# opendilab/DI-engine

Measured on NVIDIA H100. Metric: learner transitions/sec (GAE+ppo_error fwd+bwd, T=128 x B=4096 per GPU), higher is better.
Workload: dtype f32

## Files before the change

di-engine_b200/_lib.py:

```python
import ctypes
import os
from ctypes import c_double, c_int, c_longlong, c_size_t, c_void_p

_HERE = os.path.dirname(os.path.abspath(__file__))
LIB_PATH = os.environ.get("B200RL_LIB") or os.path.join(_HERE, "lib", "libb200rl.so")

P = c_void_p
LL = c_longlong
D = c_double
I = c_int

PROTOTYPES = {
    "b200rl_version": [],
    "b200rl_built_for_sm": [],
    "b200rl_workspace_bytes": [],
    "b200rl_gae": [P, P, P, P, P, P, LL, LL, LL, D, D, I, P],
    "b200rl_gae_returns": [P, P, P, P, P, LL, LL, LL, D, D, I, D, P, P, P, P, P, P, P, c_size_t, P],
    "b200rl_adv_stats": [P, LL, P, P, c_size_t, P],
    "b200rl_normalize": [P, P, LL, P, P],
    "b200rl_gae_returns_norm": [P, P, P, P, P, LL, LL, D, D, I, D, P, P, P, P, P, P, P, P, P, c_size_t, P],
    "b200rl_value_map_fwd": [I, P, LL, P, P],
    "b200rl_value_map_bwd": [I, P, P, LL, P, P],
    "b200rl_impala_mask": [P, P, P, LL, LL, P, P, P, P],
    "b200rl_ppo_fwd": [P, P, P, P, P, P, P, P, P, LL, LL, LL, D, I, D, I, P, P, P, P, c_size_t, P],
    "b200rl_ppo_bwd": [P, P, P, P, P, P, P, P, P, LL, LL, LL, D, I, D, I, P, P, P, P, P, P, P, P, P, P, P],
    "b200rl_ppo_fwd_grad": [P, P, P, P, P, P, P, P, P, LL, LL, LL, D, I, D, I, P, P, P, P, P, P, P, P, c_size_t, P],
    "b200rl_ppo_value_fwd": [P, P, P, P, LL, D, I, P, P, P, c_size_t, P],
    "b200rl_ppo_fused_supported": [P, P, P, P, P, P, P, P, P, P, LL, LL],
    "b200rl_qntd_fwd": [P, P, P, P, P, P, P, P, LL, P, LL, LL, LL, I, D, I, I, D, I, D, I, LL, D, P, P, P, P, P, P, P,
                        c_size_t, P],
    "b200rl_qntd_bwd": [P, P, P, P, P, LL, LL, LL, I, LL, I, P, P],
    "b200rl_dqfd_fwd": [P, P, P, P, P, P, P, P, P, P, P, LL, P, LL, LL, I, D, I, I, D, I, D, D, D, D, D, LL, D, P, P, P,
                        P, P, P, P, P, P, c_size_t, P],
    "b200rl_dqfd_bwd": [P, P, P, P, P, P, P, P, LL, LL, D, D, D, LL, I, P, P],
    "b200rl_soft_td_fwd": [I, P, P, P, P, P, P, P, P, LL, LL, LL, LL, I, D, D, D, I, I, D, P, P, P, P, P, P, P, P, P,
                           c_size_t, P],
    "b200rl_dntd_fwd":[P, P, P, P, P, P, P, LL, P, LL, P, LL, LL, LL, I, I, D, D, D, P, P, P, P, P, P, c_size_t, P],
    "b200rl_dntd_bwd": [P, P, P, P, LL, P, P, LL, LL, I, I, P, P],
    "b200rl_lambda_returns": [P, P, P, D, P, D, P, I, LL, LL, P, P],
    "b200rl_lambda_returns_bwd": [P, P, P, P, P, D, P, D, P, I, LL, LL, P, P, P, P, P],
    "b200rl_tb_cross_entropy_fwd": [P, P, P, LL, LL, LL, P, P],
    "b200rl_tb_cross_entropy_bwd": [P, P, P, P, LL, LL, LL, P, P],
    "b200rl_td_lambda_fwd": [P, P, P, D, D, LL, LL, P, P, P, c_size_t, P],
    "b200rl_scale": [P, P, P, LL, P],
    "b200rl_upgo_head_fwd": [P, P, P, P, P, P, LL, LL, LL, P, P, P, P, c_size_t, P],
    "b200rl_upgo_head_bwd": [P, P, P, P, P, LL, LL, LL, I, P, P],
    "b200rl_vtrace_fwd": [P, P, P, P, P, P, LL, LL, LL, D, D, D, D, D, P, P, P, P, P, c_size_t, P],
    "b200rl_vtrace_continuous_fwd": [P, P, P, P, P, P, P, P, LL, LL, LL, D, D, D, D, D, P, P, P, P, P, c_size_t, P],
    "b200rl_vtrace_continuous_bwd": [P, P, P, P, P, P, P, P, P, LL, LL, LL, P, P, P, P],
    "b200rl_vtrace_fused_supported": [P, P, P, P, P, P, LL, LL, LL, P, P],
    "b200rl_vtrace_fwd_grad": [P, P, P, P, P, P, LL, LL, LL, D, D, D, D, D, P, I, P, P, P, P, P, P, P, P, P, c_size_t, P],
    "b200rl_gae_ppo_supported": [P, P, P, P, P, LL, LL, P, P, P, P, P, P, P, P, LL, P, P],
    "b200rl_gae_ppo_fwd_grad": [P, P, P, P, P, LL, LL, D, D, I, P, P, P, P, P, P, P, P, LL, D, I, D, I, P, P, P, P, P, P,
                                P, c_size_t, P],
    "b200rl_gae_ppo_fwd_grad_dp": [P, P, P, P, P, LL, LL, D, D, I, P, P, P, P, P, P, P, P, LL, D, I, D, I, P, P, P, P, P,
                                   P, P, I, I, P, P, P, c_size_t, P],
    "b200rl_p2p_drain_mean": [P, I, I, I, P, P, P],
    "b200rl_a2c_fwd_grad": [P, P, P, P, P, P, LL, LL, P, I, P, P, P, P, P, P, P, P, P, c_size_t, P],
    "b200rl_ppo_continuous_fwd_grad": [P, P, P, P, P, P, P, P, P, P, P, P, P, LL, LL, D, I, D, I, P, I, P, P, P, P, P, P, P, P, P,
                                       P, P, c_size_t, P],
    "b200rl_a2c_continuous_fwd_grad": [P, P, P, P, P, P, P, LL, LL, P, I, P, P, P, P, P, P, P, P, P, P, c_size_t, P],
    "b200rl_grpo_fwd_grad": [I, P, P, P, P, P, P, LL, LL, LL, D, D, P, P, P, P, P, c_size_t, P],
    "b200rl_rloo_fwd_grad": [I, P, P, P, P, LL, P, LL, LL, LL, D, P, P, P, P, P, c_size_t, P],
    "b200rl_token_logp_fwd": [I, P, P, LL, LL, P, P, P],
    "b200rl_token_logp_bwd": [I, P, P, P, P, P, I, LL, LL, P, P],
    "b200rl_token_head_fwd": [P, P, P, P, P, LL, P, LL, LL, D, D, P, P, P, c_size_t, P],
    "b200rl_ppo_lm_fwd_grad": [I, P, P, P, P, P, P, LL, LL, D, D, I, I, P, P, P, P, P, P, P, P, P, c_size_t, P],
    "b200rl_ppo_lm_bwd": [I, P, P, P, LL, LL, P, P, P, P, P, P, P, P, P, P, P],
    "b200rl_a2c_lm_fwd_grad": [I, P, P, P, P, P, P, LL, LL, P, P, P, P, P, P, P, P, P, P, c_size_t, P],
    "b200rl_a2c_lm_bwd": [I, P, P, P, LL, LL, P, P, P, P, P, P, P, P, P, P, P, P],
    "b200rl_gae_ppo_set_impl": [I],
    "b200rl_vtrace_set_impl": [I],
    "b200rl_acer_policy_fwd": [P, P, P, P, P, P, LL, LL, D, P, P, P],
    "b200rl_acer_policy_bwd": [P, P, P, P, P, P, P, P, LL, LL, D, P, P],
    "b200rl_acer_value_fwd": [P, P, P, LL, LL, P, P],
    "b200rl_acer_value_bwd": [P, P, P, P, LL, LL, P, P],
    "b200rl_acer_trust_region": [P, P, LL, LL, D, P, P],
    "b200rl_ppg_bc_fwd": [P, P, P, LL, LL, P, P, P, c_size_t, P],
    "b200rl_q_retraces": [P, P, P, P, P, P, LL, LL, LL, D, P, P],
    "b200rl_quantile_td_fwd": [P, P, P, P, P, P, P, P, P, LL, LL, LL, LL, LL, LL, D, LL, LL, LL, LL, LL, LL, LL, LL, I, D, P, P,
                               P, P, P, c_size_t, P],
# ... 44 lines not shown
```

di-engine_b200/csrc/colws.cu:

```cuda
#include "../../include/b200rl.h"
#include "fused_args.cuh"

namespace b200rl {

constexpr int CW_CW = 8;
constexpr int CW_CT = CW_CW * 32;
constexpr int CW_THREADS = CW_CT + 64;
template <int TC> struct CwGeo {
    static constexpr int R = CW_CT / TC;
    static constexpr int MAX_STAGES = TC == 32 ? 8 : 4;
    static constexpr int CTAS_PER_SM = TC == 32 ? 1 : 2;
    static constexpr int PR = TC / 4;
    static constexpr int RAW_SLOTS = TC == 32 ? 4 : 2;
};
constexpr int CW_AHEAD = 2;
constexpr int CW_RAW_ARR = CW_CT * 4;
constexpr int CW_RAW_BYTES = 5 * CW_RAW_ARR;

constexpr int CW_TRACE_CHUNKS = 13;
#define CW_TRACE(slot)                                                                                   \
    do {                                                                                                 \
        if (f.trace) reinterpret_cast<unsigned long long*>(ws + 65536)[blockIdx.x * 64 + (slot)] = gtimer(); \
    } while (0)

// ... 356 lines not shown
    const long long S = a.S, L = S * a.N * 4, F = S * 4;
    const ByteSpan s[] = {byte_span(a.logit_new, L), byte_span(a.logit_old, L), byte_span(a.logit_pre, L),
                          byte_span(a.action, S * 8),   byte_span(a.value_new, F), byte_span(a.value_old, F),
                          byte_span(a.ret, F),          byte_span(a.weight, F),    byte_span(f.value, F),
                          byte_span(f.next_value, F),   byte_span(f.reward, F),    byte_span(f.done, F),
                          byte_span(f.traj, F)};
    for (const ByteSpan& x : s) *r++ = x;
    return (int)(sizeof(s) / sizeof(s[0]));
}

static int cw_writes(const FusedArgs& f, float* out, float* ws, size_t ws_bytes, ByteSpan* w) {
    const PpoArgs& a = f.p;
    const long long S = a.S, F = S * 4;
    const ByteSpan s[] = {byte_span(a.adv_out, F),
                          byte_span(a.grad_logit, S * a.N * 4),
                          byte_span(a.grad_value, F),
                          byte_span(f.mask_inplace ? f.next_value : nullptr, F),
                          byte_span(a.rec.used, 4 * sizeof(float)),
                          byte_span(ws, (long long)ws_bytes),
                          byte_span(out, 8 * sizeof(float)),
                          byte_span(f.x_seq, 24 * sizeof(unsigned int)),
                          byte_span(f.x_out_mean, 16 * sizeof(float))};
    for (const ByteSpan& x : s) *w++ = x;
    return (int)(sizeof(s) / sizeof(s[0]));
}

template <int NC, bool GRADS, int TC>
static int launch_ws(const FusedArgs& f_in, float* out, float* ws, size_t ws_bytes, cudaStream_t st) {
    FusedArgs f = f_in;
    const PpoArgs& a = f.p;
    const ChainPoint at = capture_now(st);
    ByteSpan span[16];
    f.defer_wait = !f.x_mailboxes && chain_may_defer(st, at, span, cw_early_reads(f, span));
    const int stages = cw_stages<TC>(f);
    const size_t smem = cw_smem<TC>(a.N, a.logit_pre != nullptr, a.weight != nullptr, stages);
    constexpr auto kern = gae_ppo_ws_kernel<NC, GRADS, TC>;
    int sm_count, per_sm;
    if (int rc = resident_ctas<kern>(CW_THREADS, smem, sm_count, per_sm)) return rc;
    if (per_sm > CwGeo<TC>::CTAS_PER_SM) per_sm = CwGeo<TC>::CTAS_PER_SM;
    const long long n_tiles = (f.B + TC - 1) / TC;
    long long grid = (long long)sm_count * per_sm;
    if (grid > n_tiles) grid = n_tiles;
    if (ws_bytes < WS_MIN_BYTES || !ws_partials_fit((long long)(grid * 6), ws_bytes))
        return B200RL_ERR_WORKSPACE;
    if (int rc = launch_k(kern, (int)grid, CW_THREADS, smem, st, f, ws, stages)) return rc;
    FinalizeArgs fa = ppo_finalize_args(a.S, a.logit_pre != nullptr, (int)grid);
    fa.x.mailboxes = f.x_mailboxes; fa.x.state = f.x_seq; fa.x.out_mean = f.x_out_mean; fa.x.rank = f.x_rank;
    fa.x.world = f.x_world;
    if (int rc = launch_finalize(ws, out, fa, st)) return rc;
    chain_report(st, at, true, span, cw_writes(f, out, ws, ws_bytes, span));
    return B200RL_OK;
}

static int cw_sm_count(int& n) {
    static int sms[MAX_DEVICES];
    int dev = 0;
    if (int rc = current_device(dev)) return rc;
    if (sms[dev] == 0)
        if (int rc = cuda_rc(cudaDeviceGetAttribute(&sms[dev], cudaDevAttrMultiProcessorCount, dev))) return rc;
    n = sms[dev];
    return B200RL_OK;
}

template <bool GRADS>
static int dispatch_ws(const FusedArgs& f, float* out, float* ws, size_t ws_bytes, cudaStream_t st) {
    int sm_count = 0;
    if (int rc = cw_sm_count(sm_count)) return rc;
    const int tc = cw_pick_tc(f, sm_count);
    return with_nc(f.p.N, [&](auto nc) {
        return tc == 32 ? launch_ws<nc, GRADS, 32>(f, out, ws, ws_bytes, st) : launch_ws<nc, GRADS, 16>(f, out, ws, ws_bytes, st);
    });
}

int launch_colws(const FusedArgs& f, bool grads, float* out, float* ws, size_t ws_bytes, cudaStream_t st) {
    return grads ? dispatch_ws<true>(f, out, ws, ws_bytes, st) : dispatch_ws<false>(f, out, ws, ws_bytes, st);
}

}
```

di-engine_b200/csrc/common.cuh:

```cuda
#pragma once
#include <cuda_runtime.h>
#include <stdint.h>
#include <stdlib.h>

#include <type_traits>

#define B200RL_OK 0
#ifndef B200RL_ERR_ARG
#define B200RL_ERR_ARG (-1)
#define B200RL_ERR_WORKSPACE (-2)
#endif

#define WS_CTRL_WORDS 16
#define WS_MIN_BYTES (1u << 20)

namespace b200rl {

constexpr int NUM_SMS = 132;

__device__ __forceinline__ float fmul(float a, float b) { return __fmul_rn(a, b); }
__device__ __forceinline__ float fadd(float a, float b) { return __fadd_rn(a, b); }
__device__ __forceinline__ float fsub(float a, float b) { return __fsub_rn(a, b); }

__device__ __forceinline__ float ldg_stream(const float* p) { return __ldcs(p); }
// ... 499 lines not shown
    UpstreamRecord r{};
    for (int k = 0; k < 4; ++k) r.g[k] = expected ? expected + k : nullptr;
    r.used = used;
    return r;
}

static inline UpstreamRecord verify_record(const float* g0, const float* g1, const float* g2, const float* g3,
                                           const float* used, float* hint) {
    return UpstreamRecord{{g0, g1, g2, g3}, const_cast<float*>(used), hint, 1};
}

__device__ __forceinline__ float upstream_value(const UpstreamRecord& r, unsigned owned, int k) {
    return ((owned >> k) & 1u) && r.g[k] ? *r.g[k] : 0.f;
}

template <int K>
__device__ __forceinline__ bool upstream(const UpstreamRecord& r, bool verify, unsigned owned, float (&g)[K]) {
    const bool cmp = verify && r.used != nullptr;
    bool same = cmp;
#pragma unroll
    for (int k = 0; k < K; ++k) g[k] = upstream_value(r, owned, k);
#pragma unroll
    for (int k = 0; k < K; ++k)
        if (cmp && ((owned >> k) & 1u)) same &= __float_as_uint(g[k]) == __float_as_uint(r.used[k]);
    float* rec = verify ? r.hint : r.used;
    if (rec && blockIdx.x == 0 && threadIdx.x == 0)
#pragma unroll
        for (int k = 0; k < K; ++k)
            if (!verify || ((owned >> k) & 1u)) rec[k] = g[k];
    return same;
}

static inline bool upstream_args_ok(int verify, const float* out, bool grads, bool bufs, const float* expected,
                                    const float* used) {
    return verify ? bufs : (out && (!grads || (bufs && expected && used)));
}

constexpr int MAX_DEVICES = 64;

static inline int current_device(int& dev) {
    if (int rc = cuda_rc(cudaGetDevice(&dev))) return rc;
    return (dev >= 0 && dev < MAX_DEVICES) ? B200RL_OK : B200RL_ERR_ARG;
}

template <auto K>
static inline int smem_opt_in(size_t smem) {
    static size_t opted[MAX_DEVICES];
    if (smem <= 48 * 1024) return B200RL_OK;
    int dev = 0;
    if (int rc = current_device(dev)) return rc;
    if (smem <= opted[dev]) return B200RL_OK;
    if (int rc = cuda_rc(cudaFuncSetAttribute(K, cudaFuncAttributeMaxDynamicSharedMemorySize, (int)smem))) return rc;
    opted[dev] = smem;
    return B200RL_OK;
}

template <auto K>
static inline int resident_ctas(int threads, size_t smem, int& sm_count, int& per_sm) {
    static int sms[MAX_DEVICES];
    static size_t occ_smem[MAX_DEVICES];
    static int occ[MAX_DEVICES];
    if (int rc = smem_opt_in<K>(smem)) return rc;
    int dev = 0;
    if (int rc = current_device(dev)) return rc;
    if (sms[dev] == 0)
        if (int rc = cuda_rc(cudaDeviceGetAttribute(&sms[dev], cudaDevAttrMultiProcessorCount, dev))) return rc;
    if (occ[dev] == 0 || occ_smem[dev] != smem) {
        if (int rc = cuda_rc(cudaOccupancyMaxActiveBlocksPerMultiprocessor(&occ[dev], K, threads, smem))) return rc;
        occ_smem[dev] = smem;
    }
    sm_count = sms[dev];
    per_sm = occ[dev];
    return per_sm < 1 ? B200RL_ERR_ARG : B200RL_OK;
}

template <class F>
static inline int with_nc(int n, F&& f) {
    switch (n) {
        case 2: return f(std::integral_constant<int, 2>{});
        case 3: return f(std::integral_constant<int, 3>{});
        case 4: return f(std::integral_constant<int, 4>{});
        case 5: return f(std::integral_constant<int, 5>{});
        case 6: return f(std::integral_constant<int, 6>{});
        case 7: return f(std::integral_constant<int, 7>{});
        case 8: return f(std::integral_constant<int, 8>{});
        case 9: return f(std::integral_constant<int, 9>{});
        case 10: return f(std::integral_constant<int, 10>{});
        case 12: return f(std::integral_constant<int, 12>{});
        case 14: return f(std::integral_constant<int, 14>{});
        case 16: return f(std::integral_constant<int, 16>{});
        case 18: return f(std::integral_constant<int, 18>{});
        default: return f(std::integral_constant<int, 0>{});
    }
}

struct ByteSpan {
    uintptr_t lo, hi;
};
static inline ByteSpan byte_span(const void* p, long long bytes) {
    const uintptr_t lo = reinterpret_cast<uintptr_t>(p);
    return (p && bytes > 0) ? ByteSpan{lo, lo + (uintptr_t)bytes} : ByteSpan{0, 0};
}

struct ChainPoint {
    int dev;
    bool capturing;
// ... 43 lines not shown
```

di-engine_b200/csrc/ppo.cu:

```cuda
#include "../../include/b200rl.h"
#include "ppo_math.cuh"

namespace b200rl {

template <int NC, int WHAT>
__global__ void __launch_bounds__(PPO_THREADS) ppo_tile_kernel(PpoArgs a, float* out, float* ws) {
    constexpr int PPO_R = PPO_CT;
    pdl_prologue();
    extern __shared__ __align__(128) unsigned char smem[];
    constexpr bool GRADS = (WHAT != PPO_FWD);
    constexpr bool LOSSES = (WHAT != PPO_BWD);
    const int N = NC ? NC : a.N;
    const int tid = threadIdx.x;
    const int wid = tid >> 5, lane = tid & 31;
    const bool is_producer = wid == PPO_CW;
    const bool has_pre = a.logit_pre != nullptr, has_w = a.weight != nullptr;
    const PpoTileLayout L = ppo_layout(N, has_pre, has_w, PPO_R);
    const int warp_out_bytes = 32 * N * 4;
    unsigned char* outbuf = smem + PPO_STAGES * L.stage_bytes;
    uint64_t* full = reinterpret_cast<uint64_t*>(outbuf + (GRADS ? PPO_OUTBUFS * L.logit_bytes : 0));
    uint64_t* empty = full + PPO_STAGES;

    float g[4] = {0.f, 0.f, 0.f, 0.f};
    if (GRADS && upstream<4>(a.rec, WHAT == PPO_BWD, ppo_owned(a), g)) return;
    const PpoUpstream up{g[0], g[1], g[2], g[3], 1.f / (float)a.S};

    const long long n_full = a.S / PPO_R;
    const int tail_rows = (int)(a.S - n_full * PPO_R);
    const long long n_tiles = n_full + (tail_rows ? 1 : 0);
    const int my_n = (n_tiles > blockIdx.x) ? (int)((n_tiles - blockIdx.x + gridDim.x - 1) / gridDim.x) : 0;

    if (tid == 0) {
        for (int s = 0; s < PPO_STAGES; ++s) {
            mbar_init(&full[s], 1);
            mbar_init(&empty[s], PPO_CW);
        }
        mbar_fence_init();
    }
    __syncthreads();

    float acc[6] = {0.f, 0.f, 0.f, 0.f, 0.f, 0.f};
    if (is_producer) {
        if (lane == 0) {
            for (int i = 0; i < my_n; ++i) {
                const long long t = blockIdx.x + (long long)i * gridDim.x;
                if (t >= n_full) break;
                const int sg = i % PPO_STAGES;
                if (i >= PPO_STAGES) mbar_wait(&empty[sg], (uint32_t)(((i / PPO_STAGES) - 1) & 1));
                const long long row0 = t * PPO_R;
                unsigned char* st = smem + sg * L.stage_bytes;
                uint64_t* bar = &full[sg];
                mbar_expect_tx(bar, (uint32_t)L.tx_bytes);
                tma_load_1d(st, a.logit_new + row0 * N, L.logit_bytes, bar);
                tma_load_1d(st + L.off_old, a.logit_old + row0 * N, L.logit_bytes, bar);
                if (has_pre) tma_load_1d(st + L.off_pre, a.logit_pre + row0 * N, L.logit_bytes, bar);
                tma_load_1d(st + L.off_act, a.action + row0, PPO_R * 8, bar);
                tma_load_1d(st + L.off_vn, a.value_new + row0, PPO_R * 4, bar);
                tma_load_1d(st + L.off_vo, a.value_old + row0, PPO_R * 4, bar);
                tma_load_1d(st + L.off_adv, a.adv + row0, PPO_R * 4, bar);
                tma_load_1d(st + L.off_ret, a.ret + row0, PPO_R * 4, bar);
                if (has_w) tma_load_1d(st + L.off_w, a.weight + row0, PPO_R * 4, bar);
            }
        }
    } else {
    const int rit = wid * 32 + lane;
    for (int i = 0; i < my_n; ++i) {
        const long long t = blockIdx.x + (long long)i * gridDim.x;
        const long long row0 = t * PPO_R;
        const int sg = i % PPO_STAGES;
        unsigned char* st = smem + sg * L.stage_bytes;
        const bool full_tile = t < n_full;
        if (full_tile) {
            mbar_wait(&full[sg], (uint32_t)((i / PPO_STAGES) & 1));
        } else {
            if (rit < tail_rows) {
                float* d0 = reinterpret_cast<float*>(st) + rit * N;
                float* d1 = reinterpret_cast<float*>(st + L.off_old) + rit * N;
                float* d2 = reinterpret_cast<float*>(st + L.off_pre) + rit * N;
                for (int k = 0; k < N; ++k) {
                    d0[k] = a.logit_new[(row0 + rit) * N + k];
                    d1[k] = a.logit_old[(row0 + rit) * N + k];
                    if (has_pre) d2[k] = a.logit_pre[(row0 + rit) * N + k];
                }
                reinterpret_cast<long long*>(st + L.off_act)[rit] = a.action[row0 + rit];
                reinterpret_cast<float*>(st + L.off_vn)[rit] = a.value_new[row0 + rit];
                reinterpret_cast<float*>(st + L.off_vo)[rit] = a.value_old[row0 + rit];
                reinterpret_cast<float*>(st + L.off_adv)[rit] = a.adv[row0 + rit];
                reinterpret_cast<float*>(st + L.off_ret)[rit] = a.ret[row0 + rit];
                if (has_w) reinterpret_cast<float*>(st + L.off_w)[rit] = a.weight[row0 + rit];
            }
        }
        float* gtile = reinterpret_cast<float*>(outbuf + (wid * 2 + (i & 1)) * warp_out_bytes) - wid * 32 * N;
        if (full_tile || rit < tail_rows) {
            const float adv = reinterpret_cast<const float*>(st + L.off_adv)[rit];
            ppo_row_compute<NC, LOSSES, GRADS>(a, L, st, rit, N, adv, full_tile, gtile, row0, up, acc);
        }
        if (full_tile) {
            if (GRADS) {
                fence_proxy_async_smem();
                __syncwarp();
                if (lane == 0) {
                    tma_store_1d(a.grad_logit + (row0 + wid * 32) * N, gtile + wid * 32 * N, warp_out_bytes);
                    tma_store_commit();
                    tma_store_wait_read<1>();
                }
            }
            __syncwarp();
            if (lane == 0) mbar_arrive(&empty[sg]);
        }
    }
    if (GRADS && lane == 0) tma_store_wait_read<0>();
    }
    if (LOSSES) grid_store_partials<6, PPO_THREADS>(acc, ws);
}

template <int NT, int MODE>
__global__ void __launch_bounds__(NT) ppo_fwd_kernel(PpoArgs a, float* out, float* ws) {
    pdl_prologue();
    constexpr int L = (MODE == 2) ? 32 : 1;
    const int lane = (MODE == 2) ? (threadIdx.x & 31) : 0;
    const int N = a.N, G = a.G;
    const long long per_cta = (MODE == 1) ? NT : NT / 32;
    long long s = (MODE == 1) ? (long long)blockIdx.x * NT + threadIdx.x
                              : (long long)blockIdx.x * (NT / 32) + (threadIdx.x >> 5);
    float acc[6] = {0.f, 0.f, 0.f, 0.f, 0.f, 0.f};
    for (; s < a.S; s += per_cta * gridDim.x) {
        const float* zn = a.logit_new + s * G * N;
        const float* zo = a.logit_old + s * G * N;
        const float* zp = a.logit_pre ? a.logit_pre + s * G * N : nullptr;
        float ratio_sum = 0.f, ent_sum = 0.f, akl = 0.f, kl = 0.f;
        for (int g = 0; g < G; ++g) {
            const float* rn = zn + (size_t)g * N;
            const float* ro = zo + (size_t)g * N;
            const int act = (int)a.action[s * G + g];
            float lse_n, ent;
            row_lse_entropy<L>([&](int j) { return rn[j]; }, N, lane, lse_n, ent);
            const float lse_o = row_lse<L>([&](int j) { return ro[j]; }, N, lane);
            const float lp_n = rn[act] - lse_n;
            const float lp_o = ro[act] - lse_o;
            ratio_sum += expf(lp_n - lp_o);
            ent_sum += ent;
            akl += lp_o - lp_n;
            if (zp) {
                const float* rp = zp + (size_t)g * N;
                const float lse_p = row_lse<L>([&](int j) { return rp[j]; }, N, lane);
                float dummy;
                kl += kl_term(lp_n - (rp[act] - lse_p), a.kl_type, dummy);
            }
        }
        if (lane == 0) {
            const float w = a.weight ? a.weight[s] : 1.f;
            const float adv = adv_in(a, a.adv[s]);
            const float ratio = (G == 1) ? ratio_sum : ratio_sum / (float)G;
            const float ent = (G == 1) ? ent_sum : ent_sum / (float)G;
            float dsel;
            const float sel = surrogate(ratio, adv, a.clip_lo, a.clip_hi, a.dual_clip, dsel, false, a.factor ? a.factor[s] : 1.f);
            acc[0] -= sel * w;
            float dterm;
            acc[1] += value_term(a.value_new[s], a.value_old[s], a.ret[s], a.clip, a.use_value_clip, dterm) * w;
            acc[2] += ent * w;
            acc[3] += kl;
            acc[4] += akl;
            acc[5] += (ratio > a.clip_hi || ratio < a.clip_lo) ? 1.f : 0.f;
        }
    }
    double tot[6];
// ... 57 lines not shown
        float c_act = g_pol * (-w * inv_s) * dsel * ratio_g / (float)G;
        if (zp) {
            const float* rp = zp + (size_t)g * N;
            const float lse_p = row_lse<L>([&](int j) { return rp[j]; }, N, lane);
            float dk;
            kl_term(lp_n - (rp[act] - lse_p), a.kl_type, dk);
            c_act += g_kl * dk * inv_m;
        }
        const float c_ent = g_ent * w * inv_m;
        for (int j = lane; j < N; j += L) {
            const float lp = fmaxf(rn[j] - lse_n, kF32Min);
            const float p = expf(lp);
            float gj = -c_act * p - c_ent * p * (lp + ent);
            if (j == act) gj += c_act;
            gr[j] = gj;
        }
    }
    if (lane == 0) {
        float dterm;
        value_term(a.value_new[s], a.value_old[s], a.ret[s], a.clip, a.use_value_clip, dterm);
        a.grad_value[s] = g_val * 0.5f * w * inv_s * dterm;
    }
    }
}

static bool tile_path_ok(const PpoArgs& a) {
    const bool al = aligned16(a.logit_new) && aligned16(a.logit_old) && (!a.logit_pre || aligned16(a.logit_pre)) &&
                    aligned16(a.action) && aligned16(a.value_new) && aligned16(a.value_old) && aligned16(a.adv) &&
                    aligned16(a.ret) && (!a.weight || aligned16(a.weight)) &&
                    (!a.grad_logit || aligned16(a.grad_logit));
    return a.G == 1 && a.N <= 32 && al;
}

template <int NT>
__global__ void __launch_bounds__(NT) ppo_value_kernel(const float* __restrict__ value_new,
                                                       const float* __restrict__ value_old,
                                                       const float* __restrict__ ret, const float* __restrict__ weight,
                                                       long long S, float clip, int use_clip, float* __restrict__ out,
                                                       float* __restrict__ dvalue, float* ws) {
    pdl_prologue();
    float acc[1] = {0.f};
    const float inv_s = 1.f / (float)S;
    for (long long i = (long long)blockIdx.x * NT + threadIdx.x; i < S; i += (long long)gridDim.x * NT) {
        const float w = weight ? weight[i] : 1.f;
        float d;
        const float t = value_term(value_new[i], use_clip ? value_old[i] : 0.f, ret[i], clip, use_clip, d);
        acc[0] += t * w;
        if (dvalue) dvalue[i] = 0.5f * w * inv_s * d;
    }
    double tot[1];
    if (grid_sum<1, NT>(acc, tot, ws, 0) && threadIdx.x == 0) out[0] = (float)(0.5 * tot[0] / (double)S);
}

template <int NC, int WHAT>
static int launch_tile(const PpoArgs& a, float* out, float* ws, size_t ws_bytes, cudaStream_t st) {
    constexpr int PPO_R = PPO_CT;
    const PpoTileLayout L = ppo_layout(a.N, a.logit_pre != nullptr, a.weight != nullptr, PPO_R);
    const size_t smem = (size_t)PPO_STAGES * L.stage_bytes + (WHAT != PPO_FWD ? (size_t)PPO_OUTBUFS * L.logit_bytes : 0) +
                        2 * PPO_STAGES * sizeof(uint64_t);
    constexpr auto kern = ppo_tile_kernel<NC, WHAT>;
    if (smem > 227 * 1024) return B200RL_ERR_ARG;
    int sm_count, per_sm;
    if (int rc = resident_ctas<kern>(PPO_THREADS, smem, sm_count, per_sm)) return rc;
    if (per_sm > 6) per_sm = 6;
    const long long n_tiles = (a.S + PPO_R - 1) / PPO_R;
    long long grid = (long long)sm_count * ((WHAT == PPO_BWD && a.rec.used) ? 1 : per_sm);
    if (grid > n_tiles) grid = n_tiles;
    if (WHAT != PPO_BWD && !ws_partials_fit((long long)(grid * 6), ws_bytes)) return B200RL_ERR_WORKSPACE;
    if (int rc = launch_k(kern, (int)grid, PPO_THREADS, smem, st, a, out, ws)) return rc;
    if (WHAT == PPO_BWD) return B200RL_OK;
    return launch_finalize(ws, out, ppo_finalize_args(a.S, a.logit_pre != nullptr, (int)grid), st);
}

template <int WHAT>
static int dispatch_tile(const PpoArgs& a, float* out, float* ws, size_t ws_bytes, cudaStream_t st) {
    return with_nc(a.N, [&](auto nc) { return launch_tile<nc, WHAT>(a, out, ws, ws_bytes, st); });
}

}

using namespace b200rl;

static int fill_args(PpoArgs& a, const float* logit_new, const float* logit_old, const float* logit_pretrained,
                     const long long* action, const float* value_new, const float* value_old, const float* adv,
                     const float* return_, const float* weight, long long S, long long G, long long N,
                     double clip_ratio, int use_value_clip, double dual_clip, int kl_type, const float* adv_stats,
                     const float* factor) {
    a.adv_stats = adv_stats;
    a.factor = factor;
    a.logit_new = logit_new; a.logit_old = logit_old; a.logit_pre = logit_pretrained; a.action = action;
    a.value_new = value_new; a.value_old = value_old; a.adv = adv; a.ret = return_; a.weight = weight;
    a.S = S; a.G = (int)G; a.N = (int)N; a.clip = (float)clip_ratio; a.clip_lo = (float)(1.0 - clip_ratio);
    a.clip_hi = (float)(1.0 + clip_ratio); a.dual_clip = (float)dual_clip;
    a.use_value_clip = use_value_clip; a.kl_type = kl_type;
    if (S < 0 || G < 1 || N < 1) return B200RL_ERR_ARG;
    if (!logit_new || !logit_old || !action || !value_new || !value_old || !adv || !return_) return B200RL_ERR_ARG;
    if (kl_type < 1 || kl_type > 3) return B200RL_ERR_ARG;
    return B200RL_OK;
}

extern "C" int b200rl_ppo_fwd(const float* logit_new, const float* logit_old, const float* logit_pretrained,
                              const long long* action, const float* value_new, const float* value_old,
                              const float* adv, const float* return_, const float* weight, long long S, long long G,
                              long long N, double clip_ratio, int use_value_clip, double dual_clip, int kl_type,
                              const float* adv_stats, const float* factor, float* out, float* workspace,
                              size_t workspace_bytes, void* stream) {
    PpoArgs a{};
    int rc = fill_args(a, logit_new, logit_old, logit_pretrained, action, value_new, value_old, adv, return_, weight,
                       S, G, N, clip_ratio, use_value_clip, dual_clip, kl_type, adv_stats, factor);
    if (rc != B200RL_OK || !out || !workspace) return rc != B200RL_OK ? rc : B200RL_ERR_ARG;
    if (S == 0) return B200RL_ERR_ARG;
    cudaStream_t st = (cudaStream_t)stream;
    if (tile_path_ok(a)) return dispatch_tile<PPO_FWD>(a, out, workspace, workspace_bytes, st);
    constexpr int NT = 128;
    const bool warp = a.N > 64;
    int grid = warp ? div_up(S, NT / 32) : div_up(S, NT);
    if (grid > NUM_SMS * 16) grid = NUM_SMS * 16;
    if (!ws_partials_fit((long long)((size_t)grid * 6), workspace_bytes)) return B200RL_ERR_WORKSPACE;
    if (warp) return launch_k(ppo_fwd_kernel<NT, 2>, grid, NT, 0, st, a, out, workspace);
    return launch_k(ppo_fwd_kernel<NT, 1>, grid, NT, 0, st, a, out, workspace);
}

extern "C" int b200rl_ppo_fwd_grad(const float* logit_new, const float* logit_old, const float* logit_pretrained,
                                   const long long* action, const float* value_new, const float* value_old,
// ... 9 lines not shown
    if (rc != B200RL_OK) return rc;
    if (!workspace || S == 0 || !upstream_args_ok(0, out, true, grad_logit_new && grad_value_new, g_expected, g_used))
        return B200RL_ERR_ARG;
    a.rec = forward_record(g_expected, g_used); a.grad_logit = grad_logit_new; a.grad_value = grad_value_new;
    if (!tile_path_ok(a)) return B200RL_ERR_ARG;
    return dispatch_tile<PPO_FWD_GRAD>(a, out, workspace, workspace_bytes, (cudaStream_t)stream);
}

extern "C" int b200rl_ppo_fused_supported(const float* logit_new, const float* logit_old,
                                          const float* logit_pretrained, const long long* action,
                                          const float* value_new, const float* value_old, const float* adv,
                                          const float* return_, const float* weight, const float* grad_logit_new,
                                          long long G, long long N) {
    PpoArgs a{};
    a.logit_new = logit_new; a.logit_old = logit_old; a.logit_pre = logit_pretrained; a.action = action;
    a.value_new = value_new; a.value_old = value_old; a.adv = adv; a.ret = return_; a.weight = weight;
    a.grad_logit = const_cast<float*>(grad_logit_new); a.G = (int)G; a.N = (int)N;
    return tile_path_ok(a) ? 1 : 0;
}

extern "C" int b200rl_ppo_bwd(const float* logit_new, const float* logit_old, const float* logit_pretrained,
                              const long long* action, const float* value_new, const float* value_old,
                              const float* adv, const float* return_, const float* weight, long long S, long long G,
                              long long N, double clip_ratio, int use_value_clip, double dual_clip, int kl_type,
                              const float* adv_stats, const float* factor, const float* g_policy, const float* g_value,
                              const float* g_entropy, const float* g_kl,
                              const float* g_used, float* g_hint, float* grad_logit_new, float* grad_value_new,
                              void* stream) {
    PpoArgs a{};
    int rc = fill_args(a, logit_new, logit_old, logit_pretrained, action, value_new, value_old, adv, return_, weight,
                       S, G, N, clip_ratio, use_value_clip, dual_clip, kl_type, adv_stats, factor);
    if (rc != B200RL_OK) return rc;
    if (!upstream_args_ok(1, nullptr, true, grad_logit_new && grad_value_new, nullptr, g_used)) return B200RL_ERR_ARG;
    a.rec = verify_record(g_policy, g_value, g_entropy, g_kl, g_used, g_hint);
    a.grad_logit = grad_logit_new; a.grad_value = grad_value_new;
    if (S == 0) return B200RL_OK;
    cudaStream_t st = (cudaStream_t)stream;
    constexpr int NT = 128;
    if (tile_path_ok(a)) {
        const ChainPoint at = capture_now(st);
        if (int rc = dispatch_tile<PPO_BWD>(a, nullptr, nullptr, 0, st)) return rc;
        const ByteSpan w[] = {byte_span(grad_logit_new, S * G * N * 4), byte_span(grad_value_new, S * 4),
                              byte_span(g_hint, 4 * sizeof(float))};
        chain_report(st, at, false, w, 3);
        return B200RL_OK;
    }
    if (g_used) return B200RL_ERR_ARG;
    long long grid = a.N > 64 ? div_up(S, NT / 32) : div_up(S, NT);
    if (grid > NUM_SMS * 32) grid = NUM_SMS * 32;
    if (a.N > 64) return launch_k(ppo_bwd_kernel<NT, 2>, (int)grid, NT, 0, st, a);
    return launch_k(ppo_bwd_kernel<NT, 1>, (int)grid, NT, 0, st, a);
}

extern "C" int b200rl_ppo_value_fwd(const float* value_new, const float* value_old, const float* return_,
                                    const float* weight, long long S, double clip_ratio, int use_value_clip,
                                    float* loss, float* dvalue_unit, float* workspace, size_t workspace_bytes,
                                    void* stream) {
    if (!value_new || !return_ || (use_value_clip && !value_old) || !loss || !workspace || S < 1) return B200RL_ERR_ARG;
    constexpr int NT = 256;
    long long grid = div_up(S, NT);
    if (grid > NUM_SMS * 8) grid = NUM_SMS * 8;
    if (workspace_bytes < WS_MIN_BYTES || !ws_partials_fit((long long)(grid), workspace_bytes))
        return B200RL_ERR_WORKSPACE;
    return launch_k(ppo_value_kernel<NT>, (int)grid, NT, 0, (cudaStream_t)stream, value_new, value_old, return_, weight,
                    S, (float)clip_ratio, use_value_clip, loss, dvalue_unit, workspace);
}
```

include/b200rl.h:

```cpp
#ifndef B200RL_H_
#define B200RL_H_

#include <stddef.h>

#ifdef __cplusplus
extern "C" {
#endif

#if defined(__GNUC__)
#define B200RL_API __attribute__((visibility("default")))
#else
#define B200RL_API
#endif

#define B200RL_ERR_ARG (-1)
#define B200RL_ERR_WORKSPACE (-2)

B200RL_API int b200rl_version(void);
B200RL_API int b200rl_built_for_sm(void);
B200RL_API size_t b200rl_workspace_bytes(void);

B200RL_API int b200rl_gae(const float* value, float* next_value, const float* reward, const float* done, const float* traj_flag,
               float* adv, long long T, long long C, long long A, double gamma, double lambda_,
               int mask_next_value_inplace, void* stream);

B200RL_API int b200rl_gae_returns(const float* value, float* next_value, const float* reward, const float* done,
                       const float* traj_flag, long long T, long long C, long long A, double gamma, double lambda_,
                       int mask_next_value_inplace, double value_scale, float* adv, float* unnormalized_return,
                       float* value_out, float* return_out, float* stats3, float* adv_stats2, float* workspace,
                       size_t workspace_bytes, void* stream);
B200RL_API int b200rl_adv_stats(const float* x, long long n, float* stats2, float* workspace, size_t workspace_bytes,
                     void* stream);
B200RL_API int b200rl_normalize(const float* x, const float* stats2, long long n, float* out, void* stream);

B200RL_API int b200rl_gae_returns_norm(const float* value, const float* next_value, const float* reward, const float* done,
                            const float* traj_flag, long long T, long long C, double gamma, double lambda_,
                            int value_norm, double std, const float* popart_mu, const float* popart_sigma, float* adv,
                            float* value_out, float* return_out, float* stats3, float* adv_stats2, float* scratch,
                            float* workspace, size_t workspace_bytes, void* stream);

B200RL_API int b200rl_value_map_fwd(int mode, const float* x, long long n, float* y, void* stream);
B200RL_API int b200rl_value_map_bwd(int mode, const float* x, const float* g, long long n, float* dx, void* stream);

B200RL_API int b200rl_impala_mask(const float* values, const float* rewards, const float* done, long long T, long long B,
                       float* values_out, float* rewards_out, float* weights_out, void* stream);

B200RL_API int b200rl_ppo_fwd(const float* logit_new, const float* logit_old, const float* logit_pretrained,
                   const long long* action, const float* value_new, const float* value_old, const float* adv,
                   const float* return_, const float* weight, long long S, long long G, long long N,
                   double clip_ratio, int use_value_clip, double dual_clip, int kl_type, const float* adv_stats,
                   const float* factor, float* out, float* workspace, size_t workspace_bytes, void* stream);
B200RL_API int b200rl_ppo_bwd(const float* logit_new, const float* logit_old, const float* logit_pretrained,
                   const long long* action, const float* value_new, const float* value_old, const float* adv,
                   const float* return_, const float* weight, long long S, long long G, long long N,
                   double clip_ratio, int use_value_clip, double dual_clip, int kl_type, const float* adv_stats,
                   const float* factor, const float* g_policy, const float* g_value, const float* g_entropy, const float* g_kl,
                   const float* g_used, float* g_hint, float* grad_logit_new, float* grad_value_new, void* stream);
B200RL_API int b200rl_ppo_fwd_grad(const float* logit_new, const float* logit_old, const float* logit_pretrained,
                        const long long* action, const float* value_new, const float* value_old, const float* adv,
                        const float* return_, const float* weight, long long S, long long G, long long N,
                        double clip_ratio, int use_value_clip, double dual_clip, int kl_type, const float* adv_stats,
                        const float* factor, const float* g_expected, float* g_used, float* out, float* grad_logit_new,
                        float* grad_value_new, float* workspace, size_t workspace_bytes, void* stream);
B200RL_API int b200rl_ppo_fused_supported(const float* logit_new, const float* logit_old, const float* logit_pretrained,
                               const long long* action, const float* value_new, const float* value_old,
                               const float* adv, const float* return_, const float* weight,
                               const float* grad_logit_new, long long G, long long N);

B200RL_API int b200rl_qntd_fwd(const float* q, const float* next_n_q, const long long* action, const long long* next_n_action,
                    const float* reward, const float* done, const float* weight, const float* value_gamma,
                    long long value_gamma_stride, const float* gamma_per_sample, long long S, long long G, long long N,
                    int nstep, double gamma, int cum_reward, int rescale, double rescale_eps, int criterion,
                    double criterion_param, int group_mean, long long seq_len, double priority_mix, float* loss,
                    float* td_error_per_sample, float* dcrit_saved, float* target_out, float* grad_q_unit,
                    float* priority_out, float* workspace, size_t workspace_bytes, void* stream);
B200RL_API int b200rl_qntd_bwd(const float* dcrit_saved, const float* weight, const long long* action, const float* g_loss,
                    const float* g_td, long long S, long long G, long long N, int group_mean, long long seq_len,
                    int skip_if_unit, float* grad_q, void* stream);

B200RL_API int b200rl_dqfd_fwd(const float* q, const float* next_n_q, const float* new_n_q_one_step, const long long* action,
                    const long long* next_n_action, const long long* next_n_action_one_step, const float* reward,
                    const float* done, const float* done_one_step, const float* weight, const float* value_gamma,
                    long long value_gamma_stride, const float* is_expert, long long S, long long N, int nstep,
                    double gamma, int cum_reward, int rescale, double rescale_eps, int criterion, double criterion_param,
                    double lambda_n_step_td, double lambda_one_step_td, double lambda_supervised_loss, double margin,
                    long long seq_len, double priority_mix, float* loss, float* td_error_per_sample,
                    float* loss_statistics, float* saved, float* target_n_out, float* target_1_out, float* grad_q_unit,
                    float* priority_out, float* workspace, size_t workspace_bytes, void* stream);
B200RL_API int b200rl_dqfd_bwd(const float* saved, const float* weight, const long long* action, const float* g_loss,
                    const float* g_td, const float* g_loss_statistics_n, const float* g_loss_statistics_1,
                    const float* g_loss_statistics_je, long long S, long long N, double lambda_n_step_td,
                    double lambda_one_step_td, double lambda_supervised_loss, long long seq_len, int skip_if_unit,
                    float* grad_q, void* stream);

B200RL_API int b200rl_soft_td_fwd(int mode, const float* q, const float* target_q, const float* next_q, const long long* action,
                       const float* reward, const float* done, const float* weight, const float* value_gamma,
                       long long value_gamma_stride, long long S, long long G, long long N, int nstep, double gamma,
                       double tau, double alpha, int cum_reward, int criterion, double criterion_param, float* loss,
                       float* td_error_per_sample, float* dcrit_saved, float* target_out, float* grad_q_unit,
                       float* action_gap, float* clipfrac, float* record_target_v, float* workspace,
                       size_t workspace_bytes, void* stream);

B200RL_API int b200rl_dntd_fwd(const float* dist, const float* next_n_dist, const long long* act, const long long* next_n_act,
                    const float* reward, const float* done, const float* weight, long long weight_stride,
                    const float* value_gamma, long long value_gamma_stride, const float* support, long long B,
                    long long A, long long N, int n_atom, int nstep, double gamma, double v_min, double v_max,
                    float* loss, float* td_error_per_sample, float* proj_saved, int* bad_flag, float* grad_dist_unit,
                    float* workspace, size_t workspace_bytes, void* stream);
B200RL_API int b200rl_dntd_bwd(const float* dist, const long long* act, const float* proj_saved, const float* weight,
                    long long weight_stride, const float* g_loss, const float* g_td, long long R, long long N,
                    int n_atom, int skip_if_unit, float* grad_dist, void* stream);

B200RL_API int b200rl_lambda_returns(const float* value, const float* reward, const float* gammas, double gamma,
                          const float* lambdas, double lambda_, const float* done, int upgo_mode, long long T,
                          long long B, float* ret, void* stream);
B200RL_API int b200rl_lambda_returns_bwd(const float* g_ret, const float* value, const float* reward, const float* ret,
// ... 194 lines not shown
```

Baseline: 21.31 billion.

## Restructure PPO tile kernel into one persistent CTA per SM with deep pipeline

Rewrites the PPO tile kernel so each SM runs a single persistent CTA that takes a contiguous range of tiles. Stage count is sized dynamically to fill shared memory, and the producer limits itself to a fixed prefetch distance. Gradients are written in place into the input stage buffer instead of separate output buffers, and the stage is released only after the TMA store has read it. It also adds optional per-CTA timer tracing and a geometry query API. The goal is deeper load/compute overlap and less smem overhead, but it risks lower occupancy and less latency hiding than several CTAs per SM. It is also unclear whether the workload's fused GAE+PPO path uses this kernel at all.

```diff
diff --git a/di-engine_b200/_lib.py b/di-engine_b200/_lib.py
--- a/di-engine_b200/_lib.py
+++ b/di-engine_b200/_lib.py
@@ -27,6 +27,7 @@
     "b200rl_ppo_fwd_grad": [P, P, P, P, P, P, P, P, P, LL, LL, LL, D, I, D, I, P, P, P, P, P, P, P, P, c_size_t, P],
     "b200rl_ppo_value_fwd": [P, P, P, P, LL, D, I, P, P, P, c_size_t, P],
     "b200rl_ppo_fused_supported": [P, P, P, P, P, P, P, P, P, P, LL, LL],
+    "b200rl_ppo_tile_geometry": [LL, LL, I, I, I, I, P],
     "b200rl_qntd_fwd": [P, P, P, P, P, P, P, P, LL, P, LL, LL, LL, I, D, I, I, D, I, D, I, LL, D, P, P, P, P, P, P, P,
                         c_size_t, P],
     "b200rl_qntd_bwd": [P, P, P, P, P, LL, LL, LL, I, LL, I, P, P],
diff --git a/di-engine_b200/csrc/colws.cu b/di-engine_b200/csrc/colws.cu
--- a/di-engine_b200/csrc/colws.cu
+++ b/di-engine_b200/csrc/colws.cu
@@ -432,20 +432,10 @@
     return B200RL_OK;
 }
 
-static int cw_sm_count(int& n) {
-    static int sms[MAX_DEVICES];
-    int dev = 0;
-    if (int rc = current_device(dev)) return rc;
-    if (sms[dev] == 0)
-        if (int rc = cuda_rc(cudaDeviceGetAttribute(&sms[dev], cudaDevAttrMultiProcessorCount, dev))) return rc;
-    n = sms[dev];
-    return B200RL_OK;
-}
-
 template <bool GRADS>
 static int dispatch_ws(const FusedArgs& f, float* out, float* ws, size_t ws_bytes, cudaStream_t st) {
     int sm_count = 0;
-    if (int rc = cw_sm_count(sm_count)) return rc;
+    if (int rc = sm_count_of(sm_count)) return rc;
     const int tc = cw_pick_tc(f, sm_count);
     return with_nc(f.p.N, [&](auto nc) {
         return tc == 32 ? launch_ws<nc, GRADS, 32>(f, out, ws, ws_bytes, st) : launch_ws<nc, GRADS, 16>(f, out, ws, ws_bytes, st);
diff --git a/di-engine_b200/csrc/common.cuh b/di-engine_b200/csrc/common.cuh
--- a/di-engine_b200/csrc/common.cuh
+++ b/di-engine_b200/csrc/common.cuh
@@ -575,6 +575,16 @@
     if (smem <= opted[dev]) return B200RL_OK;
     if (int rc = cuda_rc(cudaFuncSetAttribute(K, cudaFuncAttributeMaxDynamicSharedMemorySize, (int)smem))) return rc;
     opted[dev] = smem;
+    return B200RL_OK;
+}
+
+static inline int sm_count_of(int& n) {
+    static int sms[MAX_DEVICES];
+    int dev = 0;
+    if (int rc = current_device(dev)) return rc;
+    if (sms[dev] == 0)
+        if (int rc = cuda_rc(cudaDeviceGetAttribute(&sms[dev], cudaDevAttrMultiProcessorCount, dev))) return rc;
+    n = sms[dev];
     return B200RL_OK;
 }
 
diff --git a/di-engine_b200/csrc/ppo.cu b/di-engine_b200/csrc/ppo.cu
--- a/di-engine_b200/csrc/ppo.cu
+++ b/di-engine_b200/csrc/ppo.cu
@@ -3,77 +3,96 @@
 
 namespace b200rl {
 
+constexpr int PS_CW = 8;
+constexpr int PS_R = PS_CW * 32;
+constexpr int PS_THREADS = PS_R + 32;
+constexpr int PS_MAX_STAGES = 8;
+constexpr int PS_AHEAD = 2;
+constexpr size_t PS_SMEM_LIMIT = 227 * 1024 - 1024;
+constexpr int PS_TRACE_STAGES = 56;
+
 template <int NC, int WHAT>
-__global__ void __launch_bounds__(PPO_THREADS) ppo_tile_kernel(PpoArgs a, float* out, float* ws) {
-    constexpr int PPO_R = PPO_CT;
+__global__ void __launch_bounds__(PS_THREADS, 1) ppo_tile_kernel(PpoArgs a, float* ws, int n_stages, int trace) {
+    extern __shared__ __align__(128) unsigned char smem[];
+    unsigned long long* tr = trace ? reinterpret_cast<unsigned long long*>(ws + 65536) + blockIdx.x * 64 : nullptr;
+    if (tr && threadIdx.x == 0) tr[0] = gtimer();
     pdl_prologue();
-    extern __shared__ __align__(128) unsigned char smem[];
+    if (tr && threadIdx.x == 0) tr[1] = gtimer();
     constexpr bool GRADS = (WHAT != PPO_FWD);
     constexpr bool LOSSES = (WHAT != PPO_BWD);
     const int N = NC ? NC : a.N;
     const int tid = threadIdx.x;
     const int wid = tid >> 5, lane = tid & 31;
-    const bool is_producer = wid == PPO_CW;
     const bool has_pre = a.logit_pre != nullptr, has_w = a.weight != nullptr;
-    const PpoTileLayout L = ppo_layout(N, has_pre, has_w, PPO_R);
-    const int warp_out_bytes = 32 * N * 4;
-    unsigned char* outbuf = smem + PPO_STAGES * L.stage_bytes;
-    uint64_t* full = reinterpret_cast<uint64_t*>(outbuf + (GRADS ? PPO_OUTBUFS * L.logit_bytes : 0));
-    uint64_t* empty = full + PPO_STAGES;
+    const PpoTileLayout L = ppo_layout(N, has_pre, has_w, PS_R);
+    const int NS = n_stages;
+    uint64_t* full = reinterpret_cast<uint64_t*>(smem + NS * L.stage_bytes);
+    uint64_t* empty = full + PS_MAX_STAGES;
 
     float g[4] = {0.f, 0.f, 0.f, 0.f};
     if (GRADS && upstream<4>(a.rec, WHAT == PPO_BWD, ppo_owned(a), g)) return;
     const PpoUpstream up{g[0], g[1], g[2], g[3], 1.f / (float)a.S};
 
-    const long long n_full = a.S / PPO_R;
-    const int tail_rows = (int)(a.S - n_full * PPO_R);
+    const long long n_full = a.S / PS_R;
+    const int tail_rows = (int)(a.S - n_full * PS_R);
     const long long n_tiles = n_full + (tail_rows ? 1 : 0);
-    const int my_n = (n_tiles > blockIdx.x) ? (int)((n_tiles - blockIdx.x + gridDim.x - 1) / gridDim.x) : 0;
+    const long long t0 = n_tiles * blockIdx.x / gridDim.x, t1 = n_tiles * (blockIdx.x + 1) / gridDim.x;
+    const int my_n = (int)(t1 - t0);
 
     if (tid == 0) {
-        for (int s = 0; s < PPO_STAGES; ++s) {
+        for (int s = 0; s < NS; ++s) {
             mbar_init(&full[s], 1);
-            mbar_init(&empty[s], PPO_CW);
+            mbar_init(&empty[s], PS_CW);
         }
         mbar_fence_init();
     }
     __syncthreads();
 
     float acc[6] = {0.f, 0.f, 0.f, 0.f, 0.f, 0.f};
-    if (is_producer) {
+    if (wid == PS_CW) {
         if (lane == 0) {
             for (int i = 0; i < my_n; ++i) {
-                const long long t = blockIdx.x + (long long)i * gridDim.x;
+                const long long t = t0 + i;
                 if (t >= n_full) break;
-                const int sg = i % PPO_STAGES;
-                if (i >= PPO_STAGES) mbar_wait(&empty[sg], (uint32_t)(((i / PPO_STAGES) - 1) & 1));
-                const long long row0 = t * PPO_R;
+                const int sg = i % NS;
+                if (i >= NS) mbar_wait(&empty[sg], (uint32_t)(((i / NS) - 1) & 1));
+                if (NS > PS_AHEAD && i >= PS_AHEAD) {
+                    const int jb = i - PS_AHEAD;
+                    mbar_wait(&full[jb % NS], (uint32_t)((jb / NS) & 1));
+                }
+                const long long row0 = t * PS_R;
                 unsigned char* st = smem + sg * L.stage_bytes;
                 uint64_t* bar = &full[sg];
                 mbar_expect_tx(bar, (uint32_t)L.tx_bytes);
                 tma_load_1d(st, a.logit_new + row0 * N, L.logit_bytes, bar);
                 tma_load_1d(st + L.off_old, a.logit_old + row0 * N, L.logit_bytes, bar);
                 if (has_pre) tma_load_1d(st + L.off_pre, a.logit_pre + row0 * N, L.logit_bytes, bar);
-                tma_load_1d(st + L.off_act, a.action + row0, PPO_R * 8, bar);
-                tma_load_1d(st + L.off_vn, a.value_new + row0, PPO_R * 4, bar);
-                tma_load_1d(st + L.off_vo, a.value_old + row0, PPO_R * 4, bar);
-                tma_load_1d(st + L.off_adv, a.adv + row0, PPO_R * 4, bar);
-                tma_load_1d(st + L.off_ret, a.ret + row0, PPO_R * 4, bar);
-                if (has_w) tma_load_1d(st + L.off_w, a.weight + row0, PPO_R * 4, bar);
+                tma_load_1d(st + L.off_act, a.action + row0, PS_R * 8, bar);
+                tma_load_1d(st + L.off_vn, a.value_new + row0, PS_R * 4, bar);
+                tma_load_1d(st + L.off_vo, a.value_old + row0, PS_R * 4, bar);
+                tma_load_1d(st + L.off_adv, a.adv + row0, PS_R * 4, bar);
+                tma_load_1d(st + L.off_ret, a.ret + row0, PS_R * 4, bar);
+                if (has_w) tma_load_1d(st + L.off_w, a.weight + row0, PS_R * 4, bar);
             }
         }
     } else {
-    const int rit = wid * 32 + lane;
-    for (int i = 0; i < my_n; ++i) {
-        const long long t = blockIdx.x + (long long)i * gridDim.x;
-        const long long row0 = t * PPO_R;
-        const int sg = i % PPO_STAGES;
-        unsigned char* st = smem + sg * L.stage_bytes;
-        const bool full_tile = t < n_full;
-        if (full_tile) {
-            mbar_wait(&full[sg], (uint32_t)((i / PPO_STAGES) & 1));
-        } else {
-            if (rit < tail_rows) {
+        const int rit = wid * 32 + lane;
+        const int warp_out_bytes = 32 * N * 4;
+        for (int i = 0; i < my_n; ++i) {
+            const long long t = t0 + i;
+            const long long row0 = t * PS_R;
+            const int sg = i % NS;
+            unsigned char* st = smem + sg * L.stage_bytes;
+            const bool full_tile = t < n_full;
+            if (full_tile) {
+                mbar_wait(&full[sg], (uint32_t)((i / NS) & 1));
+                if (tr && tid == 0) {
+                    const unsigned long long now = gtimer();
+                    if (i == 0) tr[2] = now;
+                    tr[3] = now;
+                    if (i < PS_TRACE_STAGES) tr[8 + i] = now;
+                }
+            } else if (rit < tail_rows) {
                 float* d0 = reinterpret_cast<float*>(st) + rit * N;
                 float* d1 = reinterpret_cast<float*>(st + L.off_old) + rit * N;
                 float* d2 = reinterpret_cast<float*>(st + L.off_pre) + rit * N;
@@ -89,29 +108,39 @@
                 reinterpret_cast<float*>(st + L.off_ret)[rit] = a.ret[row0 + rit];
                 if (has_w) reinterpret_cast<float*>(st + L.off_w)[rit] = a.weight[row0 + rit];
             }
-        }
-        float* gtile = reinterpret_cast<float*>(outbuf + (wid * 2 + (i & 1)) * warp_out_bytes) - wid * 32 * N;
-        if (full_tile || rit < tail_rows) {
-            const float adv = reinterpret_cast<const float*>(st + L.off_adv)[rit];
-            ppo_row_compute<NC, LOSSES, GRADS>(a, L, st, rit, N, adv, full_tile, gtile, row0, up, acc);
-        }
-        if (full_tile) {
+            if (full_tile || rit < tail_rows) {
+                const float adv = reinterpret_cast<const float*>(st + L.off_adv)[rit];
+                ppo_row_compute<NC, LOSSES, GRADS>(a, L, st, rit, N, adv, full_tile, reinterpret_cast<float*>(st), row0,
+                                                   up, acc);
+            }
+            if (!full_tile) continue;
             if (GRADS) {
                 fence_proxy_async_smem();
                 __syncwarp();
                 if (lane == 0) {
-                    tma_store_1d(a.grad_logit + (row0 + wid * 32) * N, gtile + wid * 32 * N, warp_out_bytes);
+                    tma_store_1d(a.grad_logit + (row0 + wid * 32) * N, st + wid * warp_out_bytes, warp_out_bytes);
                     tma_store_commit();
-                    tma_store_wait_read<1>();
+                    if (NS == 1) {
+                        tma_store_wait_read<0>();
+                        mbar_arrive(&empty[sg]);
+                    } else {
+                        tma_store_wait_read<1>();
+                        if (i > 0) mbar_arrive(&empty[(i - 1) % NS]);
+                    }
                 }
+                __syncwarp();
+            } else {
+                __syncwarp();
+                if (lane == 0) mbar_arrive(&empty[sg]);
             }
-            __syncwarp();
-            if (lane == 0) mbar_arrive(&empty[sg]);
-        }
-    }
-    if (GRADS && lane == 0) tma_store_wait_read<0>();
-    }
-    if (LOSSES) grid_store_partials<6, PPO_THREADS>(acc, ws);
+        }
+        if (GRADS && lane == 0) tma_store_wait_read<0>();
+    }
+    if (LOSSES) grid_store_partials<6, PS_THREADS>(acc, ws);
+    if (tr && tid == 0) {
+        tr[4] = gtimer();
+        tr[5] = (unsigned long long)smid() << 32 | (unsigned long long)my_n;
+    }
 }
 
 template <int NT, int MODE>
@@ -275,24 +304,39 @@
     if (grid_sum<1, NT>(acc, tot, ws, 0) && threadIdx.x == 0) out[0] = (float)(0.5 * tot[0] / (double)S);
 }
 
+struct PsGeo {
+    int grid, stages;
+    size_t smem;
+};
+static PsGeo ps_pick(long long S, int N, bool has_pre, bool has_w, bool verify_only, int sm_count) {
+    PsGeo g{};
+    const size_t stage = (size_t)ppo_layout(N, has_pre, has_w, PS_R).stage_bytes;
+    const size_t bars = 2 * PS_MAX_STAGES * sizeof(uint64_t);
+    const long long n_tiles = (S + PS_R - 1) / PS_R;
+    g.grid = (int)(n_tiles < sm_count ? n_tiles : sm_count);
+    const long long per_cta = g.grid > 0 ? (n_tiles + g.grid - 1) / g.grid : 0;
+    long long stages = verify_only ? 1 : (long long)((PS_SMEM_LIMIT - bars) / stage);
+    if (stages > PS_MAX_STAGES) stages = PS_MAX_STAGES;
+    if (stages > per_cta) stages = per_cta;
+    g.stages = stages < 1 ? 0 : (int)stages;
+    g.smem = (size_t)g.stages * stage + bars;
+    return g;
+}
+
 template <int NC, int WHAT>
 static int launch_tile(const PpoArgs& a, float* out, float* ws, size_t ws_bytes, cudaStream_t st) {
-    constexpr int PPO_R = PPO_CT;
-    const PpoTileLayout L = ppo_layout(a.N, a.logit_pre != nullptr, a.weight != nullptr, PPO_R);
-    const size_t smem = (size_t)PPO_STAGES * L.stage_bytes + (WHAT != PPO_FWD ? (size_t)PPO_OUTBUFS * L.logit_bytes : 0) +
-                        2 * PPO_STAGES * sizeof(uint64_t);
+    int sm_count = 0;
+    if (int rc = sm_count_of(sm_count)) return rc;
+    const PsGeo g = ps_pick(a.S, a.N, a.logit_pre != nullptr, a.weight != nullptr, WHAT == PPO_BWD && a.rec.used, sm_count);
+    if (g.stages < 1) return B200RL_ERR_ARG;
     constexpr auto kern = ppo_tile_kernel<NC, WHAT>;
-    if (smem > 227 * 1024) return B200RL_ERR_ARG;
-    int sm_count, per_sm;
-    if (int rc = resident_ctas<kern>(PPO_THREADS, smem, sm_count, per_sm)) return rc;
-    if (per_sm > 6) per_sm = 6;
-    const long long n_tiles = (a.S + PPO_R - 1) / PPO_R;
-    long long grid = (long long)sm_count * ((WHAT == PPO_BWD && a.rec.used) ? 1 : per_sm);
-    if (grid > n_tiles) grid = n_tiles;
-    if (WHAT != PPO_BWD && !ws_partials_fit((long long)(grid * 6), ws_bytes)) return B200RL_ERR_WORKSPACE;
-    if (int rc = launch_k(kern, (int)grid, PPO_THREADS, smem, st, a, out, ws)) return rc;
+    if (int rc = smem_opt_in<kern>(g.smem)) return rc;
+    if (WHAT != PPO_BWD && !ws_partials_fit((long long)g.grid * 6, ws_bytes)) return B200RL_ERR_WORKSPACE;
+    const int trace = WHAT != PPO_BWD && trace_enabled();
+    if (trace && (size_t)65536 * 4 + (size_t)g.grid * 64 * 8 > ws_bytes) return B200RL_ERR_WORKSPACE;
+    if (int rc = launch_k(kern, g.grid, PS_THREADS, g.smem, st, a, ws, g.stages, trace)) return rc;
     if (WHAT == PPO_BWD) return B200RL_OK;
-    return launch_finalize(ws, out, ppo_finalize_args(a.S, a.logit_pre != nullptr, (int)grid), st);
+    return launch_finalize(ws, out, ppo_finalize_args(a.S, a.logit_pre != nullptr, g.grid), st);
 }
 
 template <int WHAT>
@@ -408,6 +452,14 @@
     return launch_k(ppo_bwd_kernel<NT, 1>, (int)grid, NT, 0, st, a);
 }
 
+extern "C" int b200rl_ppo_tile_geometry(long long S, long long N, int has_pretrained, int has_weight, int verify_only,
+                                        int sm_count, long long* geometry3) {
+    if (S < 1 || N < 1 || N > 32 || sm_count < 1 || !geometry3) return B200RL_ERR_ARG;
+    const PsGeo g = ps_pick(S, (int)N, has_pretrained != 0, has_weight != 0, verify_only != 0, sm_count);
+    geometry3[0] = g.grid; geometry3[1] = g.stages; geometry3[2] = (long long)g.smem;
+    return B200RL_OK;
+}
+
 extern "C" int b200rl_ppo_value_fwd(const float* value_new, const float* value_old, const float* return_,
                                     const float* weight, long long S, double clip_ratio, int use_value_clip,
                                     float* loss, float* dvalue_unit, float* workspace, size_t workspace_bytes,
diff --git a/include/b200rl.h b/include/b200rl.h
--- a/include/b200rl.h
+++ b/include/b200rl.h
@@ -62,6 +62,8 @@
                         double clip_ratio, int use_value_clip, double dual_clip, int kl_type, const float* adv_stats,
                         const float* factor, const float* g_expected, float* g_used, float* out, float* grad_logit_new,
                         float* grad_value_new, float* workspace, size_t workspace_bytes, void* stream);
+B200RL_API int b200rl_ppo_tile_geometry(long long S, long long N, int has_pretrained, int has_weight, int verify_only,
+                                        int sm_count, long long* geometry3);
 B200RL_API int b200rl_ppo_fused_supported(const float* logit_new, const float* logit_old, const float* logit_pretrained,
                                const long long* action, const float* value_new, const float* value_old,
                                const float* adv, const float* return_, const float* weight,
```

Result: faster. 22.42 billion, median of 6 (+5.2%).
